# XShengTech/gpu-docker-api

Hardware: AMD Instinct MI355X
Metric: p50 replicaSet create->running + patch(GPU rescale) latency (lower is better)
Workload: dtype n/a; 1 GPU; global_batch=1, seq_len=0, parallelism=1 concurrent tenants, 1 daemon, 1 GPUs, patch=gpuCount 1->0

## Files before the change

### __graft_entry__.py

```python
from __future__ import annotations


def build() -> None:
    from gpu_docker_api_amd.ops import build as ops_build

    artifacts = ops_build.build_all()
    for name, path in artifacts.items():
        print(f"built {name}: {path}")

    import gpu_docker_api_amd
    from gpu_docker_api_amd.routers.app import build_app
    from gpu_docker_api_amd.ops import iocopy

    assert iocopy.uring_available() or True
    print("package import OK")


def smoke() -> None:
    import asyncio

    import torch

    assert torch.cuda.is_available(), "smoke() needs a GPU"

    from gpu_docker_api_amd.ops import hipcore

    ext = hipcore.load_ext()
    n = ext.device_count()
    assert n >= 1, "no HIP devices"
    info = ext.device_info(0)
    print(f"GPU0: {info['name']} ({info['gcnArchName']}), "
          f"{info['totalGlobalMem'] / 2**30:.0f} GiB")

    def err_over_bound(C, A64, B64, ref=None):
        if ref is None:
            ref = A64 @ B64
        bound = A64.shape[1] * 2.0 ** -23 * (A64.abs() @ B64.abs())
# ... 98 lines not shown
```

### gpu_docker_api_amd/ops/__init__.py

```python
"""Native ops: HIP/CDNA4 kernels and the io_uring copy engine.

Built in-tree by :mod:`.build` (the .so files live next to this file so they
travel to GPU boxes with the repo snapshot). On a GPU box these MUST load —
ops fail loudly rather than falling back to a silent eager path.
"""
```

### gpu_docker_api_amd/ops/build.py

```python
from __future__ import annotations

import os
import subprocess
import sys
import sysconfig

ROOT = os.path.dirname(os.path.dirname(os.path.dirname(os.path.abspath(__file__))))
CSRC = os.path.join(ROOT, "csrc")
OPS = os.path.join(ROOT, "gpu_docker_api_amd", "ops")
BIN = os.path.join(CSRC, "bin")
HIPCC = os.environ.get("HIPCC", "/opt/rocm/bin/hipcc")
ARCH = os.environ.get("PYTORCH_ROCM_ARCH", "gfx950")


def _newer(out: str, *srcs: str) -> bool:
    if not os.path.exists(out):
        return False
    omt = os.path.getmtime(out)
    return all(os.path.getmtime(s) <= omt for s in srcs)


def _run(cmd: list[str]) -> None:
    print("+", " ".join(cmd), flush=True)
    subprocess.run(cmd, check=True)
# ... 47 lines not shown
    src = os.path.join(CSRC, "iocopy.cpp")
    out = os.path.join(OPS, "_iocopy.so")
    if not force and _newer(out, src):
        return out
    import pybind11

    py_inc = sysconfig.get_paths()["include"]
    cmd = [
        "g++",
        "-O2",
        "-std=c++17",
        "-fPIC",
        "-shared",
        src,
        "-o",
        out,
        f"-I{pybind11.get_include()}",
        f"-I{py_inc}",
    ]
    _run(cmd)
    return out


def build_rccl_smoke(force: bool = False) -> str:
    src = os.path.join(CSRC, "rccl_smoke.hip")
    out = os.path.join(BIN, "rccl_smoke")
    if not force and _newer(out, src):
        return out
    os.makedirs(BIN, exist_ok=True)
    cmd = [
        HIPCC,
        f"--offload-arch={ARCH}",
        "-O2",
        "-std=c++17",
        src,
        "-o",
        out,
        "-I/opt/rocm/include",
        "-L/opt/rocm/lib",
        "-lrccl",
    ]
    _run(cmd)
    return out


def build_all(force: bool = False) -> dict:
    return {
        "iocopy": build_iocopy(force),
        "hipcore": build_hipcore(force),
        "rccl_smoke": build_rccl_smoke(force),
    }


if __name__ == "__main__":
    force = "--force" in sys.argv
    for name, path in build_all(force).items():
        print(f"built {name}: {path}")
```

### gpu_docker_api_amd/runtime/proc.py

```python
from __future__ import annotations

import asyncio
import json
import logging
import os
import shutil
import signal
import subprocess
import time
import uuid as uuidlib
from typing import Dict, List, Optional

from ..models.etcd import ContainerSpec
from ..utils.names import safe_subpath
from ..xerrors import ContainerExisted, ContainerNotExist, VolumeExisted
from .base import ContainerState, GpuResolver, RuntimeDriver, VolumeState
from .devices import visible_device_env

log = logging.getLogger(__name__)

CGROUP_ROOT = "/sys/fs/cgroup"
DEFAULT_CMD = ["sleep", "infinity"]


class _Proc:
    def __init__(self, state: ContainerState, spec: ContainerSpec) -> None:
        self.state = state
        self.spec = spec
        self.popen: Optional[subprocess.Popen] = None
        self.cgroup: Optional[str] = None
        self.restart_policy: str = (
            (spec.host_config.get("RestartPolicy") or {}).get("Name", "") or "no"
        )
        self.manually_stopped = False
        self.restarts = 0
        self.next_restart_at = 0.0
        self.last_start_at = 0.0
        self.attached_pid = 0
        self.attached_start = 0
        self.was_started = False
        self.start_ticks = 0


class ProcRuntime(RuntimeDriver):
    owns_rootfs = True

    def __init__(
        self,
        base_dir: str = "",
        gpu_resolver: Optional[GpuResolver] = None,
        use_cgroups: bool = True,
        loop_volumes: bool = False,
    ) -> None:
        self.base = base_dir or os.path.join(os.getcwd(), ".state", "procrt")
        for sub in ("containers", "volumes", "images", "trash"):
            os.makedirs(os.path.join(self.base, sub), exist_ok=True)
        self.gpu_resolver: GpuResolver = gpu_resolver or (lambda _u: None)
        self.use_cgroups = use_cgroups
        self.loop_volumes = loop_volumes
        self._procs: Dict[str, _Proc] = {}
        self.volumes: Dict[str, VolumeState] = {}
        self._supervisor: Optional[asyncio.Task] = None

        self._load_volumes()
        self._load_containers()
        try:
            asyncio.get_running_loop()
            if self._procs:
                self._ensure_supervisor()
        except RuntimeError:
            pass

    def _ensure_supervisor(self) -> None:
        if self._supervisor is None or self._supervisor.done():
            self._supervisor = asyncio.get_running_loop().create_task(
                self._supervise_loop()
# ... 95 lines not shown

    def _leader_pid(self, p: _Proc) -> int:
        if p.popen is not None:
            return p.popen.pid
        return p.attached_pid

    def _refresh(self, p: _Proc) -> None:
        if p.state.running and not self._alive(p):
            p.state.running = False
            p.state.status = "exited"
            p.state.pid = 0
            p.attached_pid = 0
            self._write_meta(p)

    def _write_meta(self, p: _Proc) -> None:
        try:
            meta = {
                "id": p.state.id,
                "pid": self._leader_pid(p) if p.state.running else 0,
                "starttime": p.start_ticks if p.state.running else 0,
                "running": p.state.running,
                "restarts": p.restarts,
            }
            with open(os.path.join(self._cdir(p.state.name), "meta.json"), "w") as f:
                json.dump(meta, f)
        except OSError:
            pass

    def _load_containers(self) -> None:
        trash = os.path.join(self.base, "trash")
        for entry in os.listdir(trash):
            shutil.rmtree(os.path.join(trash, entry), ignore_errors=True)
        croot = os.path.join(self.base, "containers")
        for name in sorted(os.listdir(croot)):
            if ".deleting-" in name:
                shutil.rmtree(os.path.join(croot, name), ignore_errors=True)
                continue
            specf = os.path.join(croot, name, "spec.json")
            if not os.path.isfile(specf):
                continue
            try:
                spec = ContainerSpec.deserialize(open(specf).read())
            except Exception:
                continue
            meta = {}
            try:
                meta = json.load(open(os.path.join(croot, name, "meta.json")))
            except Exception:
# ... 22 lines not shown
                    p.start_ticks = p.attached_start
                    p.was_started = True
                    p.last_start_at = time.monotonic()
                    st.pid = pid
                    st.running = True
                    state_char = self._proc_stat(pid)[0]
                    if state_char in ("T", "t"):
                        st.paused, st.status = True, "paused"
                    else:
                        st.status = "running"
                else:
                    p.restarts = 0
                    p.was_started = True
                    p.manually_stopped = False
            else:
                p.manually_stopped = True
            self._procs[name] = p

    async def create(self, spec: ContainerSpec) -> str:
        name = spec.container_name
        if name in self._procs:
            raise ContainerExisted(name)
        cid = uuidlib.uuid4().hex[:12]
        rootfs = os.path.join(self._cdir(name), "rootfs")
        os.makedirs(rootfs, exist_ok=True)
        seed = self._image_dir(spec.image) if spec.image else ""
        if seed and os.path.isdir(seed):
            await asyncio.get_running_loop().run_in_executor(
                None, lambda: shutil.copytree(seed, rootfs, dirs_exist_ok=True)
            )
        binds = list(spec.host_config.get("Binds") or [])
        for b in binds:
            src, _, dest = b.partition(":")
            dest = dest.split(":")[0]
            if not src or not dest:
                continue
            vol = self.volumes.get(src)
            src_path = vol.mountpoint if vol else src
            link = os.path.join(rootfs, dest.lstrip("/"))
            os.makedirs(os.path.dirname(link), exist_ok=True)
            if not os.path.lexists(link):
                os.symlink(src_path, link)
        st = ContainerState(
            id=cid,
            name=name,
            image=spec.image,
            status="created",
            env=list(spec.env),
            gpu_uuids=list(spec.gpu_uuids),
            cpuset_cpus=spec.cpuset_cpus,
            memory=spec.memory_bytes,
            port_bindings=dict(spec.host_config.get("PortBindings") or {}),
            upper_dir=rootfs,
            binds=binds,
        )
        p = _Proc(st, spec)
        self._procs[name] = p
        with open(os.path.join(self._cdir(name), "spec.json"), "w") as f:
            f.write(spec.serialize())
        return cid

    def _get(self, name: str) -> _Proc:
        if name not in self._procs:
            raise ContainerNotExist(name)
        return self._procs[name]

    _base_env: Optional[Dict[str, str]] = None

    def _env_for(self, p: _Proc) -> Dict[str, str]:
        if ProcRuntime._base_env is None:
            ProcRuntime._base_env = dict(os.environ)
        env = dict(ProcRuntime._base_env)
        env.update(visible_device_env(p.state.gpu_uuids, self.gpu_resolver))
        for e in p.state.env:
            k, _, v = e.partition("=")
            env[k] = v
        return env

    @staticmethod
    def _enable_controllers(path: str) -> None:
        ctrl_file = os.path.join(path, "cgroup.subtree_control")
        avail_file = os.path.join(path, "cgroup.controllers")
        try:
            with open(avail_file) as f:
                avail = set(f.read().split())
            want = [c for c in ("memory", "cpuset") if c in avail]
            for c in want:
                try:
                    with open(ctrl_file, "w") as f:
                        f.write(f"+{c}")
                except OSError:
                    pass
        except OSError:
            pass

    def _setup_cgroup(self, name: str, p: _Proc, pid: int) -> None:
        if not self.use_cgroups:
            return
        parent = os.path.join(CGROUP_ROOT, "gda")
        cg = os.path.join(parent, name)
# ... 9 lines not shown
                with open(os.path.join(cg, "cpuset.cpus"), "w") as f:
                    f.write(p.state.cpuset_cpus)
            mems = p.spec.host_config.get("CpusetMems", "")
            if mems:
                try:
                    with open(os.path.join(cg, "cpuset.mems"), "w") as f:
                        f.write(mems)
                except OSError:
                    pass
            with open(os.path.join(cg, "cgroup.procs"), "w") as f:
                f.write(str(pid))
            p.cgroup = cg
        except OSError:
            p.cgroup = None

    async def start(self, name: str) -> None:
        p = self._get(name)
        self._refresh(p)
        p.manually_stopped = False
        self._ensure_supervisor()
        if p.state.running:
            return
        cmd = list(p.spec.config.get("Cmd") or []) or DEFAULT_CMD
        logf = open(os.path.join(self._cdir(name), "console.log"), "ab")
        try:
            p.popen = subprocess.Popen(
                cmd,
                cwd=p.state.upper_dir,
                env=self._env_for(p),
                stdout=logf,
                stderr=subprocess.STDOUT,
                start_new_session=True,
            )
        finally:
            logf.close()
        p.attached_pid = 0
        p.was_started = True
        p.last_start_at = time.monotonic()
        p.start_ticks = self._proc_starttime(p.popen.pid) or 0
        p.state.pid = p.popen.pid
        p.state.running, p.state.paused, p.state.status = True, False, "running"
        self._setup_cgroup(name, p, p.popen.pid)
        self._write_meta(p)

    def _signal_group(self, p: _Proc, sig: int) -> None:
        if not self._alive(p):
            return
        try:
            os.killpg(os.getpgid(self._leader_pid(p)), sig)
        except ProcessLookupError:
            pass

    async def stop(self, name: str, timeout: int = 10, _removing: bool = False) -> None:
        p = self._get(name)
        p.manually_stopped = True
        self._refresh(p)
        if self._alive(p):
            self._signal_group(p, signal.SIGTERM)
            self._signal_group(p, signal.SIGCONT)
            spin_until = time.monotonic() + 0.002
            while time.monotonic() < spin_until and self._alive(p):
                await asyncio.sleep(0)
            deadline = time.monotonic() + timeout
            delay = 0.001
            while time.monotonic() < deadline and self._alive(p):
                await asyncio.sleep(delay)
                delay = min(delay * 2, 0.02)
            if self._alive(p):
                self._signal_group(p, signal.SIGKILL)
                kill_deadline = time.monotonic() + 5
                while time.monotonic() < kill_deadline and self._alive(p):
                    await asyncio.sleep(0.005)
        leader = self._leader_pid(p)
        if leader:
            try:
                os.killpg(leader, signal.SIGKILL)
            except (ProcessLookupError, PermissionError):
                pass
        p.state.running, p.state.paused, p.state.status = False, False, "exited"
        p.state.pid = 0
        p.attached_pid = 0
        if not _removing:
            self._write_meta(p)

    async def pause(self, name: str) -> None:
        p = self._get(name)
        if p.cgroup:
            try:
                with open(os.path.join(p.cgroup, "cgroup.freeze"), "w") as f:
                    f.write("1")
                p.state.paused, p.state.status = True, "paused"
                return
            except OSError:
                pass
        self._signal_group(p, signal.SIGSTOP)
        p.state.paused, p.state.status = True, "paused"

    async def unpause(self, name: str) -> None:
        p = self._get(name)
        if p.cgroup:
            try:
                with open(os.path.join(p.cgroup, "cgroup.freeze"), "w") as f:
                    f.write("0")
                p.state.paused, p.state.status = False, "running"
                return
            except OSError:
                pass
        self._signal_group(p, signal.SIGCONT)
        p.state.paused, p.state.status = False, "running"

    async def restart(self, name: str, timeout: int = 10) -> None:
        await self.stop(name, timeout)
        await self.start(name)

    async def remove(self, name: str, force: bool = True) -> None:
        p = self._get(name)
        self._refresh(p)
        if p.state.running:
            if not force:
                raise RuntimeError(f"{name} is running")
            await self.stop(name, timeout=2, _removing=True)
        if p.cgroup:
            try:
                os.rmdir(p.cgroup)
            except OSError:
                pass
        self._procs.pop(name, None)
        cdir = self._cdir(name)
        shutil.rmtree(cdir, ignore_errors=True)

    async def inspect(self, name: str) -> Optional[ContainerState]:
        p = self._procs.get(name)
        if p is None:
            return None
        self._refresh(p)
        return p.state

    async def list(self, all: bool = True) -> List[ContainerState]:
        for p in self._procs.values():
            self._refresh(p)
        return [p.state for p in self._procs.values() if all or p.state.running]

    async def execute_rc(self, name: str, cmd: List[str], workdir: str = ""):
        p = self._get(name)
        self._refresh(p)
        if not p.state.running:
            raise RuntimeError(f"{name} is not running")
        cwd = (
            os.path.join(p.state.upper_dir, workdir.lstrip("/"))
            if workdir
            else p.state.upper_dir
        )
# ... 172 lines not shown
```

### gpu_docker_api_amd/services/replicaset.py

```python
from __future__ import annotations

import asyncio
import logging
import os
import shutil
from typing import Dict, List, Optional, Tuple

from ..config import Config
from ..models import ContainerCommit, ContainerExecute, ContainerRun, PatchRequest
from ..models.etcd import ContainerSpec, HistoryItem, _now_str
from ..models.memory import to_bytes
from ..parallel import CpuScheduler, GpuScheduler, PortScheduler
from ..runtime.base import ContainerState, RuntimeDriver
from ..state.keys import Resource
from ..state.store import StateStore
from ..state.workqueue import WorkQueue
from ..utils.copy import CopyEngine
from ..utils.names import safe_subpath
from ..utils.timing import PhaseTimer
from ..state.keys import RELEASED_SET_KEY
from ..version import MergeMap, ReleasedSet, VersionMap
from ..xerrors import (
    ContainerExisted,
    ContainerNotExist,
    NoPatchRequired,
    NoRollbackRequired,
)
from .saga import Saga

log = logging.getLogger(__name__)


def versioned(name: str, version: int) -> str:
    return f"{name}-{version}"


class ReplicaSetService:
    def __init__(
        self,
        *,
# ... 252 lines not shown
        vname_old: str,
        timer: PhaseTimer,
        migrate_src: Optional[str] = None,
    ) -> Tuple[str, str]:
        old_state = await self.runtime.inspect(vname_old)
        cid, vname_new = await self._run_container(saga, name, spec, only_create=True, timer=timer)
        new_state = await self.runtime.inspect(vname_new)
        src = migrate_src or (old_state.upper_dir if old_state is not None else "")
        if (
            new_state is not None
            and src
            and new_state.upper_dir
            and os.path.isdir(src)
        ):
            await self.copy.copy_dir(src, new_state.upper_dir)
        timer.mark("copy")
        await self.runtime.start(vname_new)
        timer.mark("start")
        if old_state is not None and old_state.upper_dir and os.path.isdir(old_state.upper_dir):
            merge_path = safe_subpath(self.cfg.merges_dir, name, vname_old)
            try:
                if getattr(self.runtime, "owns_rootfs", False):
                    os.makedirs(os.path.dirname(merge_path), exist_ok=True)
                    shutil.rmtree(merge_path, ignore_errors=True)
                    try:
                        os.rename(old_state.upper_dir, merge_path)
                    except OSError:
                        os.makedirs(merge_path, exist_ok=True)
                        await self.copy.copy_dir(old_state.upper_dir, merge_path)
                else:
                    os.makedirs(merge_path, exist_ok=True)
                    await self.copy.copy_dir(old_state.upper_dir, merge_path)
                self.merges.set(vname_old, merge_path)
                self._prune_merge_layers(name)
            except Exception:
                log.exception("preserving %s layer failed", vname_old)
        timer.mark("preserve")
        if old_state is not None:
            self.ports.restore(self._host_ports(old_state))
            await self.runtime.remove(vname_old, force=True)
        self._released.discard(vname_old)
        timer.mark("delete_old")
        return vname_new, cid

    def _prune_merge_layers(self, name: str) -> None:
        keep = self.cfg.keep_merge_layers
        if keep <= 0:
            return
        prefix = name + "-"
        entries = []
        for vname, path in self.merges.snapshot().items():
            if vname.startswith(prefix):
                try:
                    entries.append((int(vname[len(prefix):]), vname, path))
                except ValueError:
                    continue
        entries.sort(reverse=True)
        for _v, vname, path in entries[keep:]:
            self.merges.remove(vname)
            shutil.rmtree(path, ignore_errors=True)

    @staticmethod
    def _host_ports(state: ContainerState) -> List[int]:
        out: List[int] = []
        for _cport, bindings in (state.port_bindings or {}).items():
            for b in bindings or []:
                try:
                    out.append(int(b.get("HostPort", "0")))
                except (TypeError, ValueError):
                    continue
        return [p for p in out if p]

    async def rollback_container(
        self, name: str, target_version: int, restore_data: bool = False
    ) -> Dict:
        timer = PhaseTimer("replicaset.rollback")
        cur_version = self.versions.get(name)
        if cur_version is None:
            raise ContainerNotExist(name)
        if cur_version == target_version:
            raise NoRollbackRequired(name)
        target = await self._spec_at_version(name, target_version)
        live = await self._load_spec(name)
# ... 194 lines not shown
```

### gpu_docker_api_amd/utils/files.py

```python
from __future__ import annotations

import os


def dir_size(path: str) -> int:
    total = 0
    for root, _dirs, files in os.walk(path):
        for f in files:
            fp = os.path.join(root, f)
            try:
                st = os.lstat(fp)
            except OSError:
                continue
            blocks = getattr(st, "st_blocks", None)
            total += blocks * 512 if blocks is not None else st.st_size
    return total


def is_dir(path: str) -> bool:
    return os.path.isdir(path)
```

Measured before the change: 3.846 ms.

## Move container process lifecycle to native vfork/pidfd module

Adds a pybind11 C++ module that spawns container processes with vfork/execve using a pre-encoded base environment, exposes a pidfd, and provides native tree removal and container-dir preparation. Stop now waits on the pidfd through the event loop instead of sleep-polling, and rmtree calls go through the native remover. The aim is to cut subprocess.Popen fork/exec overhead, polling latency and Python filesystem walking on the create and rescale path. It adds a native build dependency and subtle signal, fd and orphan-reaping logic. Pause also gains a short wait for the stopped state, which may add latency.

```diff
diff --git a/__graft_entry__.py b/__graft_entry__.py
--- a/__graft_entry__.py
+++ b/__graft_entry__.py
@@ -10,9 +10,10 @@
 
     import gpu_docker_api_amd
     from gpu_docker_api_amd.routers.app import build_app
-    from gpu_docker_api_amd.ops import iocopy
+    from gpu_docker_api_amd.ops import iocopy, proclife
 
     assert iocopy.uring_available() or True
+    assert proclife.available(), "native lifecycle module did not load"
     print("package import OK")
 
 
diff --git a/csrc/proclife.cpp b/csrc/proclife.cpp
--- /dev/null
+++ b/csrc/proclife.cpp
@@ -0,0 +1,151 @@
+#include <pybind11/pybind11.h>
+#include <pybind11/stl.h>
+
+#include <cstdio>
+#include <memory>
+
+#include "proclife_core.h"
+
+namespace py = pybind11;
+namespace pl = proclife;
+
+namespace {
+
+pl::BaseEnv g_base_env;
+
+std::string fsbytes(py::handle h, const char* what) {
+  PyObject* raw = nullptr;
+  if (!PyUnicode_FSConverter(h.ptr(), &raw)) throw py::error_already_set();
+  py::bytes b = py::reinterpret_steal<py::bytes>(raw);
+  std::string s = b;
+  if (s.find('\0') != std::string::npos)
+    throw py::value_error(std::string("embedded null byte in ") + what);
+  return s;
+}
+
+std::vector<pl::KV> env_items(py::handle mapping) {
+  std::vector<pl::KV> out;
+  if (mapping.is_none()) return out;
+  py::object items = py::isinstance<py::dict>(mapping)
+                         ? py::reinterpret_borrow<py::dict>(mapping).attr("items")()
+                         : py::reinterpret_borrow<py::object>(mapping);
+  for (py::handle it : items) {
+    py::tuple kv = py::reinterpret_borrow<py::tuple>(it);
+    std::string k = fsbytes(kv[0], "environment");
+    if (k.find('=') != std::string::npos)
+      throw py::value_error("illegal environment variable name");
+    out.emplace_back(std::move(k), fsbytes(kv[1], "environment"));
+  }
+  return out;
+}
+
+[[noreturn]] void raise_oserror(int err, const std::string& filename) {
+  errno = err;
+  if (filename.empty())
+    PyErr_SetFromErrno(PyExc_OSError);
+  else
+    PyErr_SetFromErrnoWithFilename(PyExc_OSError, filename.c_str());
+  throw py::error_already_set();
+}
+
+class PyChild {
+ public:
+  explicit PyChild(pl::Child&& c) : c_(std::move(c)), pid_(c_.pid) {}
+
+  int pid() const { return pid_; }
+  unsigned long long starttime() const { return c_.starttime; }
+  py::object returncode() const {
+    return c_.exited ? py::cast(c_.returncode) : py::none();
+  }
+  py::object poll() {
+    return c_.poll() ? py::cast(c_.returncode) : py::none();
+  }
+  py::object wait(py::object timeout) {
+    int ms = timeout.is_none() ? -1 : static_cast<int>(timeout.cast<double>() * 1000.0);
+    bool done;
+    {
+      py::gil_scoped_release nogil;
+      done = c_.wait(ms);
+    }
+    return done ? py::cast(c_.returncode) : py::none();
+  }
+  int fileno() const { return c_.pidfd; }
+  void close() { c_.close_fd(); }
+
+ private:
+  pl::Child c_;
+  int pid_;
+};
+
+std::unique_ptr<PyChild> spawn(py::sequence argv, py::object cwd, py::object env_overrides,
+                               py::object log_path) {
+  std::vector<std::string> args;
+  for (py::handle a : argv) args.push_back(fsbytes(a, "argv"));
+  if (args.empty()) throw py::value_error("empty argv");
+  std::string cwd_s = fsbytes(cwd, "cwd"), log_s = fsbytes(log_path, "log_path");
+  std::vector<pl::KV> over = env_items(env_overrides);
+  pl::Child child;
+  pl::SpawnError res;
+  {
+    py::gil_scoped_release nogil;
+    res = pl::spawn(args, cwd_s, g_base_env, over, log_s, &child);
+  }
+  if (res.err) raise_oserror(res.err, res.filename);
+  return std::make_unique<PyChild>(std::move(child));
+}
+
+}
+
+PYBIND11_MODULE(_proclife, m) {
+  m.doc() = "container process lifecycle on raw syscalls (csrc/proclife_core.h)";
+
+  py::class_<PyChild>(m, "Child")
+      .def_property_readonly("pid", &PyChild::pid)
+      .def_property_readonly("starttime", &PyChild::starttime)
+      .def_property_readonly("returncode", &PyChild::returncode)
+      .def("poll", &PyChild::poll)
+      .def("wait", &PyChild::wait, py::arg("timeout") = py::none())
+      .def("fileno", &PyChild::fileno)
+      .def("close", &PyChild::close);
+
+  m.def(
+      "set_base_env",
+      [](py::object mapping) {
+        g_base_env.set(env_items(mapping));
+        return g_base_env.size();
+      },
+      py::arg("env"), "snapshot and encode the base environment once");
+  m.def("base_env_size", [] { return g_base_env.size(); });
+  m.def("spawn", &spawn, py::arg("argv"), py::arg("cwd"), py::arg("env_overrides"),
+        py::arg("log_path"));
+  m.def("proc_starttime", [](int pid) { return pl::read_starttime(pid); }, py::arg("pid"));
+  m.def(
+      "remove_tree",
+      [](py::object path) {
+        std::string p = fsbytes(path, "path");
+        long failed;
+        {
+          py::gil_scoped_release nogil;
+          failed = pl::remove_tree(p.c_str());
+        }
+        return failed;
+      },
+      py::arg("path"));
+  m.def(
+      "prepare_container_dir",
+      [](py::object cdir, py::object spec_json) {
+        std::string d = fsbytes(cdir, "cdir"), failed;
+        std::string data = spec_json.cast<std::string>();
+        if (int e = pl::prepare_container_dir(d, data.data(), data.size(), &failed))
+          raise_oserror(e, failed);
+      },
+      py::arg("cdir"), py::arg("spec_json"));
+  m.def(
+      "write_file",
+      [](py::object path, py::object data) {
+        std::string p = fsbytes(path, "path");
+        std::string d = data.cast<std::string>();
+        if (int e = pl::write_file(p.c_str(), d.data(), d.size())) raise_oserror(e, p);
+      },
+      py::arg("path"), py::arg("data"));
+}
diff --git a/csrc/proclife_core.h b/csrc/proclife_core.h
--- /dev/null
+++ b/csrc/proclife_core.h
@@ -0,0 +1,515 @@
+#pragma once
+
+#ifndef _GNU_SOURCE
+#define _GNU_SOURCE
+#endif
+
+#include <cerrno>
+#include <cstdio>
+#include <csignal>
+#include <cstdlib>
+#include <cstring>
+#include <mutex>
+#include <string>
+#include <unordered_map>
+#include <utility>
+#include <vector>
+
+#include <dirent.h>
+#include <fcntl.h>
+#include <poll.h>
+#include <sys/stat.h>
+#include <sys/syscall.h>
+#include <sys/types.h>
+#include <sys/wait.h>
+#include <unistd.h>
+
+namespace proclife {
+
+using KV = std::pair<std::string, std::string>;
+
+
+class BaseEnv {
+ public:
+  void set(const std::vector<KV>& kv) {
+    entries_.clear();
+    index_.clear();
+    entries_.reserve(kv.size());
+    for (const auto& e : kv) {
+      auto it = index_.find(e.first);
+      if (it == index_.end()) {
+        index_.emplace(e.first, entries_.size());
+        entries_.push_back(e.first + "=" + e.second);
+      } else {
+        entries_[it->second] = e.first + "=" + e.second;
+      }
+    }
+  }
+  size_t size() const { return entries_.size(); }
+  const std::vector<std::string>& entries() const { return entries_; }
+  long find(const std::string& key) const {
+    auto it = index_.find(key);
+    return it == index_.end() ? -1 : static_cast<long>(it->second);
+  }
+
+ private:
+  std::vector<std::string> entries_;
+  std::unordered_map<std::string, size_t> index_;
+};
+
+class MergedEnv {
+ public:
+  MergedEnv(const BaseEnv& base, const std::vector<KV>& overrides) {
+    const auto& be = base.entries();
+    slots_.reserve(be.size() + overrides.size() + 1);
+    for (const auto& s : be) slots_.push_back(s.c_str());
+    owned_.reserve(overrides.size());
+    std::vector<std::pair<const std::string*, size_t>> added;
+    for (const auto& o : overrides) {
+      owned_.push_back(o.first + "=" + o.second);
+      const char* entry = owned_.back().c_str();
+      long at = base.find(o.first);
+      if (at < 0) {
+        for (const auto& a : added)
+          if (*a.first == o.first) at = static_cast<long>(a.second);
+      }
+      if (at >= 0) {
+        slots_[static_cast<size_t>(at)] = entry;
+      } else {
+        added.emplace_back(&o.first, slots_.size());
+        slots_.push_back(entry);
+      }
+    }
+    slots_.push_back(nullptr);
+  }
+  char* const* envp() const { return const_cast<char* const*>(slots_.data()); }
+  const char* get(const char* key) const {
+    size_t n = std::strlen(key);
+    for (const char* e : slots_)
+      if (e && std::strncmp(e, key, n) == 0 && e[n] == '=') return e + n + 1;
+    return nullptr;
+  }
+
+ private:
+  std::vector<std::string> owned_;
+  std::vector<const char*> slots_;
+};
+
+
+inline unsigned long long read_starttime(pid_t pid, char* state_out = nullptr) {
+  char path[48];
+  std::snprintf(path, sizeof path, "/proc/%d/stat", static_cast<int>(pid));
+  int fd = ::open(path, O_RDONLY | O_CLOEXEC);
+  if (fd < 0) return 0;
+  char buf[2048];
+  size_t len = 0;
+  for (;;) {
+    ssize_t n = ::read(fd, buf + len, sizeof buf - 1 - len);
+    if (n < 0 && errno == EINTR) continue;
+    if (n <= 0) break;
+    len += static_cast<size_t>(n);
+    if (len == sizeof buf - 1) break;
+  }
+  ::close(fd);
+  buf[len] = '\0';
+  const char* after = nullptr;
+  for (size_t i = 0; i + 1 < len; ++i)
+    if (buf[i] == ')' && buf[i + 1] == ' ') after = buf + i + 2;
+  if (!after) return 0;
+  char state = *after;
+  if (state_out) *state_out = state;
+  if (state == 'Z' || state == 'X' || state == '\0') return 0;
+  const char* p = after;
+  for (int field = 0; field < 19; ++field) {
+    while (*p && *p != ' ' && *p != '\n') ++p;
+    while (*p == ' ') ++p;
+    if (!*p) return 0;
+  }
+  char* end = nullptr;
+  errno = 0;
+  unsigned long long v = std::strtoull(p, &end, 10);
+  if (end == p || errno) return 0;
+  return v;
+}
+
+
+#ifndef P_PIDFD
+#define P_PIDFD 3
+#endif
+
+namespace detail {
+inline std::mutex& orphan_mu() {
+  static std::mutex m;
+  return m;
+}
+inline std::vector<pid_t>& orphans() {
+  static std::vector<pid_t> v;
+  return v;
+}
+inline void reap_orphans() {
+  std::lock_guard<std::mutex> g(orphan_mu());
+  auto& v = orphans();
+  for (size_t i = 0; i < v.size();) {
+    int st;
+    pid_t r = ::waitpid(v[i], &st, WNOHANG);
+    if (r == v[i] || (r < 0 && errno == ECHILD)) {
+      v[i] = v.back();
+      v.pop_back();
+    } else {
+      ++i;
+    }
+  }
+}
+}
+
+struct Child {
+  pid_t pid = -1;
+  int pidfd = -1;
+  unsigned long long starttime = 0;
+  bool exited = false;
+  int returncode = 0;
+
+  Child() = default;
+  Child(const Child&) = delete;
+  Child& operator=(const Child&) = delete;
+  Child(Child&& o) noexcept { *this = std::move(o); }
+  Child& operator=(Child&& o) noexcept {
+    if (this != &o) {
+      release();
+      pid = o.pid, pidfd = o.pidfd, starttime = o.starttime;
+      exited = o.exited, returncode = o.returncode;
+      o.pid = -1, o.pidfd = -1, o.exited = true;
+    }
+    return *this;
+  }
+  ~Child() { release(); }
+
+  bool poll() {
+    if (exited || pid <= 0) return exited;
+    siginfo_t info;
+    for (;;) {
+      std::memset(&info, 0, sizeof info);
+      int r = pidfd >= 0
+                  ? ::waitid(static_cast<idtype_t>(P_PIDFD), static_cast<id_t>(pidfd), &info,
+                             WEXITED | WNOHANG)
+                  : ::waitid(P_PID, static_cast<id_t>(pid), &info, WEXITED | WNOHANG);
+      if (r == 0) break;
+      if (errno == EINTR) continue;
+      exited = true;
+      returncode = 0;
+      return true;
+    }
+    if (info.si_pid == 0) return false;
+    exited = true;
+    returncode = info.si_code == CLD_EXITED ? info.si_status : -info.si_status;
+    return true;
+  }
+
+  bool wait(int timeout_ms) {
+    if (poll()) return true;
+    if (pidfd >= 0) {
+      struct pollfd pfd = {pidfd, POLLIN, 0};
+      for (;;) {
+        int r = ::poll(&pfd, 1, timeout_ms);
+        if (r < 0 && errno == EINTR) continue;
+        break;
+      }
+      return poll();
+    }
+    for (int waited = 0; timeout_ms < 0 || waited < timeout_ms; ++waited) {
+      if (poll()) return true;
+      ::usleep(1000);
+    }
+    return poll();
+  }
+
+  void close_fd() {
+    if (pidfd >= 0) {
+      ::close(pidfd);
+      pidfd = -1;
+    }
+  }
+
+  void release() {
+    if (pid > 0 && !exited && !poll()) {
+      std::lock_guard<std::mutex> g(detail::orphan_mu());
+      detail::orphans().push_back(pid);
+    }
+    close_fd();
+    pid = -1;
+  }
+};
+
+
+struct SpawnError {
+  int err = 0;
+  std::string filename;
+};
+
+namespace detail {
+
+#ifndef SYS_close_range
+#define SYS_close_range 436
+#endif
+
+struct ChildPlan {
+  int logfd;
+  const char* cwd;
+  char* const* argv;
+  char* const* envp;
+  const char* const* candidates;
+  const sigset_t* sigmask;
+  int max_fd;
+  volatile int* err;
+  volatile int* stage;
+};
+
+[[noreturn]] __attribute__((noinline)) inline void child_exec(const ChildPlan& p) {
+  struct sigaction dfl;
+  std::memset(&dfl, 0, sizeof dfl);
+  dfl.sa_handler = SIG_DFL;
+  for (int sig = 1; sig < NSIG; ++sig) {
+    struct sigaction cur;
+    if (::sigaction(sig, nullptr, &cur) != 0 || cur.sa_handler == SIG_DFL) continue;
+    if (cur.sa_handler == SIG_IGN && sig != SIGPIPE && sig != SIGXFSZ) continue;
+    ::sigaction(sig, &dfl, nullptr);
+  }
+  int stage = 3;
+  do {
+    if (::setsid() < 0) break;
+    if (::dup2(p.logfd, 1) < 0 || ::dup2(p.logfd, 2) < 0) break;
+    stage = 1;
+    if (::chdir(p.cwd) != 0) break;
+    stage = 3;
+    if (::sigprocmask(SIG_SETMASK, p.sigmask, nullptr) != 0) break;
+    if (::syscall(SYS_close_range, 3U, ~0U, 0U) != 0)
+      for (int fd = 3; fd < p.max_fd; ++fd) ::close(fd);
+    stage = 2;
+    int saved = 0;
+    for (const char* const* c = p.candidates; *c; ++c) {
+      ::execve(*c, p.argv, p.envp);
+      if (errno != ENOENT && errno != ENOTDIR && saved == 0) saved = errno;
+    }
+    if (saved) errno = saved;
+  } while (false);
+  *p.err = errno ? errno : EINVAL;
+  *p.stage = stage;
+  ::_exit(127);
+}
+
+__attribute__((noinline)) inline pid_t vfork_child(const ChildPlan& plan, int* vfork_errno) {
+  pid_t pid = ::vfork();
+  if (pid == 0) child_exec(plan);
+  *vfork_errno = errno;
+  return pid;
+}
+
+}
+
+inline SpawnError spawn(const std::vector<std::string>& argv, const std::string& cwd,
+                        const BaseEnv& base, const std::vector<KV>& overrides,
+                        const std::string& log_path, Child* out) {
+  SpawnError res;
+  if (argv.empty()) {
+    res.err = EINVAL;
+    return res;
+  }
+  detail::reap_orphans();
+  MergedEnv env(base, overrides);
+
+  std::vector<char*> cargv;
+  cargv.reserve(argv.size() + 1);
+  for (const auto& a : argv) cargv.push_back(const_cast<char*>(a.c_str()));
+  cargv.push_back(nullptr);
+
+  std::vector<std::string> cands;
+  int skipped_err = ENOENT;
+  const std::string& name = argv[0];
+  if (name.find('/') != std::string::npos) {
+    cands.push_back(name);
+  } else {
+    const char* path = env.get("PATH");
+    std::string dirs = path ? path : "/bin:/usr/bin";
+    for (size_t pos = 0;;) {
+      size_t colon = dirs.find(':', pos);
+      std::string dir = dirs.substr(pos, colon == std::string::npos ? colon : colon - pos);
+      std::string cand = dir.empty() ? name : dir + "/" + name;
+      std::string probe = cand[0] == '/' ? cand : cwd + "/" + cand;
+      struct stat st;
+      if (::stat(probe.c_str(), &st) != 0 && (errno == ENOENT || errno == ENOTDIR))
+        skipped_err = errno;
+      else
+        cands.push_back(std::move(cand));
+      if (colon == std::string::npos) break;
+      pos = colon + 1;
+    }
+  }
+  std::vector<const char*> cptrs;
+  cptrs.reserve(cands.size() + 1);
+  for (const auto& c : cands) cptrs.push_back(c.c_str());
+  cptrs.push_back(nullptr);
+
+  int logfd = ::open(log_path.c_str(), O_WRONLY | O_CREAT | O_APPEND | O_CLOEXEC, 0666);
+  if (logfd < 0) {
+    res.err = errno, res.filename = log_path;
+    return res;
+  }
+  if (logfd < 3) {
+    int moved = ::fcntl(logfd, F_DUPFD_CLOEXEC, 3);
+    int e = errno;
+    ::close(logfd);
+    if (moved < 0) {
+      res.err = e, res.filename = log_path;
+      return res;
+    }
+    logfd = moved;
+  }
+
+  volatile int child_err = 0, child_stage = 0;
+  pid_t pid = -1;
+  int err = 0;
+  if (cands.empty()) {
+    struct stat st;
+    if (::stat(cwd.c_str(), &st) != 0) {
+      err = errno, child_stage = 1;
+    } else {
+      err = skipped_err, child_stage = 2;
+    }
+  } else {
+    long open_max = ::sysconf(_SC_OPEN_MAX);
+    sigset_t all, old;
+    sigfillset(&all);
+    pthread_sigmask(SIG_SETMASK, &all, &old);
+    detail::ChildPlan plan = {logfd,        cwd.c_str(), cargv.data(),
+                              env.envp(),   cptrs.data(), &old,
+                              open_max > 0 && open_max < 65536 ? static_cast<int>(open_max) : 65536,
+                              &child_err,   &child_stage};
+    int vfork_err = 0;
+    pid = detail::vfork_child(plan, &vfork_err);
+    pthread_sigmask(SIG_SETMASK, &old, nullptr);
+    if (pid < 0) {
+      err = vfork_err, child_stage = 3;
+    } else if (child_err != 0) {
+      err = child_err;
+      int st;
+      while (::waitpid(pid, &st, 0) < 0 && errno == EINTR) {
+      }
+    }
+  }
+  ::close(logfd);
+
+  if (err != 0) {
+    res.err = err;
+    res.filename = child_stage == 1 ? cwd : child_stage == 2 ? argv[0] : std::string();
+    return res;
+  }
+  Child c;
+  c.pid = pid;
+  c.pidfd = static_cast<int>(::syscall(SYS_pidfd_open, pid, 0));
+  c.starttime = read_starttime(pid);
+  *out = std::move(c);
+  return res;
+}
+
+
+namespace detail {
+
+constexpr int kDirFlags = O_RDONLY | O_DIRECTORY | O_NOFOLLOW | O_CLOEXEC;
+
+inline long empty_dir(int dfd) {
+  DIR* d = ::fdopendir(dfd);
+  if (!d) {
+    ::close(dfd);
+    return 1;
+  }
+  std::vector<std::pair<std::string, unsigned char>> names;
+  for (;;) {
+    errno = 0;
+    struct dirent* e = ::readdir(d);
+    if (!e) break;
+    const char* n = e->d_name;
+    if (n[0] == '.' && (n[1] == '\0' || (n[1] == '.' && n[2] == '\0'))) continue;
+    names.emplace_back(n, e->d_type);
+  }
+  long failed = errno ? 1 : 0;
+  for (auto& ent : names) {
+    const char* n = ent.first.c_str();
+    bool is_dir = ent.second == DT_DIR;
+    if (ent.second == DT_UNKNOWN) {
+      struct stat st;
+      is_dir = ::fstatat(dfd, n, &st, AT_SYMLINK_NOFOLLOW) == 0 && S_ISDIR(st.st_mode);
+    }
+    if (is_dir) {
+      int sub = ::openat(dfd, n, kDirFlags);
+      if (sub < 0) {
+        ++failed;
+        continue;
+      }
+      failed += empty_dir(sub);
+      if (::unlinkat(dfd, n, AT_REMOVEDIR) != 0) ++failed;
+    } else if (::unlinkat(dfd, n, 0) != 0) {
+      ++failed;
+    }
+  }
+  ::closedir(d);
+  return failed;
+}
+
+}
+
+inline long remove_tree(const char* path) {
+  int dfd = ::open(path, detail::kDirFlags);
+  if (dfd < 0) return errno == ENOENT ? 0 : 1;
+  long failed = detail::empty_dir(dfd);
+  if (::rmdir(path) != 0) ++failed;
+  return failed;
+}
+
+
+inline int write_file(const char* path, const char* data, size_t len) {
+  int fd = ::open(path, O_WRONLY | O_CREAT | O_TRUNC | O_CLOEXEC, 0666);
+  if (fd < 0) return errno;
+  while (len > 0) {
+    ssize_t n = ::write(fd, data, len);
+    if (n < 0) {
+      if (errno == EINTR) continue;
+      int e = errno;
+      ::close(fd);
+      return e;
+    }
+    data += n, len -= static_cast<size_t>(n);
+  }
+  return ::close(fd) != 0 ? errno : 0;
+}
+
+inline int make_dirs(const std::string& path) {
+  if (::mkdir(path.c_str(), 0777) == 0) return 0;
+  if (errno == EEXIST) {
+    struct stat st;
+    return (::stat(path.c_str(), &st) == 0 && S_ISDIR(st.st_mode)) ? 0 : EEXIST;
+  }
+  if (errno != ENOENT) return errno;
+  size_t end = path.find_last_not_of('/');
+  size_t slash = end == std::string::npos ? end : path.rfind('/', end);
+  if (slash == std::string::npos || slash == 0) return ENOENT;
+  if (int e = make_dirs(path.substr(0, slash))) return e;
+  if (::mkdir(path.c_str(), 0777) == 0 || errno == EEXIST) return 0;
+  return errno;
+}
+
+inline int prepare_container_dir(const std::string& cdir, const char* spec, size_t len,
+                                 std::string* failed) {
+  std::string rootfs = cdir + "/rootfs";
+  if (int e = make_dirs(rootfs)) {
+    *failed = rootfs;
+    return e;
+  }
+  std::string specf = cdir + "/spec.json";
+  if (int e = write_file(specf.c_str(), spec, len)) {
+    *failed = specf;
+    return e;
+  }
+  return 0;
+}
+
+}
diff --git a/csrc/proclife_selftest.cpp b/csrc/proclife_selftest.cpp
--- /dev/null
+++ b/csrc/proclife_selftest.cpp
@@ -0,0 +1,217 @@
+#include <cstdio>
+#include <cstdlib>
+#include <fstream>
+#include <sstream>
+
+#include "proclife_core.h"
+
+namespace pl = proclife;
+
+static int g_failed = 0;
+#define CHECK(cond)                                                        \
+  do {                                                                     \
+    if (!(cond)) {                                                         \
+      std::fprintf(stderr, "FAIL %s:%d: %s\n", __FILE__, __LINE__, #cond); \
+      ++g_failed;                                                          \
+    }                                                                      \
+  } while (0)
+
+static int count_fds() {
+  DIR* d = ::opendir("/proc/self/fd");
+  if (!d) return -1;
+  int n = 0;
+  while (struct dirent* e = ::readdir(d))
+    if (e->d_name[0] != '.') ++n;
+  ::closedir(d);
+  return n - 1;
+}
+
+static bool have_children() {
+  siginfo_t info;
+  std::memset(&info, 0, sizeof info);
+  return ::waitid(P_ALL, 0, &info, WEXITED | WNOHANG | WNOWAIT) == 0;
+}
+
+static std::string slurp(const std::string& path) {
+  std::ifstream f(path);
+  std::stringstream ss;
+  ss << f.rdbuf();
+  return ss.str();
+}
+
+static void build_tree(const std::string& root) {
+  CHECK(pl::make_dirs(root + "/a/b/c") == 0);
+  CHECK(pl::write_file((root + "/a/f1").c_str(), "x", 1) == 0);
+  CHECK(pl::write_file((root + "/a/b/f2").c_str(), "yy", 2) == 0);
+  CHECK(::link((root + "/a/f1").c_str(), (root + "/a/b/c/hard").c_str()) == 0);
+  CHECK(::symlink("/nonexistent/target", (root + "/a/dangling").c_str()) == 0);
+  CHECK(pl::write_file((root + "/locked").c_str(), "z", 1) == 0);
+  CHECK(::chmod((root + "/locked").c_str(), 0) == 0);
+}
+
+int main() {
+  char tmpl[] = "/tmp/proclife-selftest-XXXXXX";
+  const char* made = ::mkdtemp(tmpl);
+  if (!made) {
+    std::perror("mkdtemp");
+    return 2;
+  }
+  const std::string top = made;
+
+  pl::BaseEnv base;
+  base.set({{"PATH", "/usr/local/bin:/usr/bin:/bin"}, {"KEEP", "1"}, {"OVER", "base"}});
+
+  { pl::Child warm; }
+  const int fds_before = count_fds();
+  CHECK(!have_children());
+
+  {
+    pl::MergedEnv env(base, {{"OVER", "a=b"}, {"NEW", ""}, {"NEW", "last"}, {"OVER", "final"}});
+    CHECK(std::string(env.get("OVER")) == "final");
+    CHECK(std::string(env.get("NEW")) == "last");
+    CHECK(std::string(env.get("KEEP")) == "1");
+    CHECK(env.get("ABSENT") == nullptr);
+    int n = 0;
+    for (char* const* e = env.envp(); *e; ++e) ++n;
+    CHECK(n == 4);
+  }
+
+  for (int round = 0; round < 200; ++round) {
+    const std::string cdir = top + "/c" + std::to_string(round);
+    std::string failed;
+    CHECK(pl::prepare_container_dir(cdir, "{}", 2, &failed) == 0);
+    pl::Child c;
+    pl::SpawnError e = pl::spawn({"sleep", "30"}, cdir + "/rootfs", base,
+                                 {{"ROUND", std::to_string(round)}}, cdir + "/console.log", &c);
+    CHECK(e.err == 0);
+    if (e.err) break;
+    CHECK(c.pid > 0 && c.pidfd >= 0 && c.starttime > 0);
+    CHECK(::getsid(c.pid) == c.pid && ::getpgid(c.pid) == c.pid);
+    CHECK(!c.poll());
+    CHECK(pl::read_starttime(c.pid) == c.starttime);
+    if (round % 3 == 0) {
+      CHECK(::kill(-c.pid, SIGKILL) == 0);
+    } else {
+      CHECK(::kill(-c.pid, round % 2 ? SIGTERM : SIGKILL) == 0);
+      CHECK(c.wait(5000));
+      CHECK(c.returncode == (round % 2 ? -SIGTERM : -SIGKILL));
+      CHECK(c.poll() && c.poll());
+      c.close_fd();
+      c.close_fd();
+    }
+    CHECK(pl::remove_tree(cdir.c_str()) == 0);
+    struct stat st;
+    CHECK(::lstat(cdir.c_str(), &st) != 0 && errno == ENOENT);
+  }
+
+  {
+    const std::string cdir = top + "/out";
+    std::string failed;
+    CHECK(pl::prepare_container_dir(cdir, "{}", 2, &failed) == 0);
+    for (int i = 0; i < 2; ++i) {
+      pl::Child c;
+      pl::SpawnError e = pl::spawn({"sh", "-c", "echo out; echo err >&2; exit 7"}, cdir + "/rootfs",
+                                   base, {}, cdir + "/console.log", &c);
+      CHECK(e.err == 0);
+      CHECK(c.wait(5000) && c.returncode == 7);
+    }
+    CHECK(slurp(cdir + "/console.log") == "out\nerr\nout\nerr\n");
+    CHECK(pl::remove_tree(cdir.c_str()) == 0);
+  }
+
+  {
+    const std::string cdir = top + "/bad";
+    std::string failed;
+    CHECK(pl::prepare_container_dir(cdir, "{}", 2, &failed) == 0);
+    CHECK(pl::write_file((cdir + "/rootfs/noexec").c_str(), "#!/bin/sh\n", 10) == 0);
+    CHECK(::chmod((cdir + "/rootfs/noexec").c_str(), 0644) == 0);
+    for (int round = 0; round < 200; ++round) {
+      pl::Child c;
+      pl::SpawnError e;
+      switch (round % 5) {
+        case 0:
+          e = pl::spawn({"definitely-not-a-command"}, cdir + "/rootfs", base, {},
+                        cdir + "/console.log", &c);
+          CHECK(e.err == ENOENT);
+          break;
+        case 1:
+          e = pl::spawn({"./noexec"}, cdir + "/rootfs", base, {}, cdir + "/console.log", &c);
+          CHECK(e.err == EACCES);
+          break;
+        case 2:
+          e = pl::spawn({"/no/such/binary"}, cdir + "/rootfs", base, {}, cdir + "/console.log", &c);
+          CHECK(e.err == ENOENT);
+          break;
+        case 3:
+          e = pl::spawn({"sleep", "1"}, cdir + "/missing-cwd", base, {}, cdir + "/console.log", &c);
+          CHECK(e.err == ENOENT && e.filename == cdir + "/missing-cwd");
+          break;
+        default:
+          e = pl::spawn({"sleep", "1"}, cdir + "/rootfs", base, {}, cdir + "/no-dir/console.log",
+                        &c);
+          CHECK(e.err == ENOENT);
+          break;
+      }
+      CHECK(c.pid == -1 && c.pidfd == -1);
+    }
+    CHECK(pl::remove_tree(cdir.c_str()) == 0);
+  }
+
+  for (int round = 0; round < 50; ++round) {
+    const std::string root = top + "/tree";
+    build_tree(root);
+    CHECK(pl::remove_tree(root.c_str()) == 0);
+    struct stat st;
+    CHECK(::lstat(root.c_str(), &st) != 0);
+  }
+  {
+    const std::string outside = top + "/outside", root = top + "/tree2";
+    CHECK(pl::make_dirs(outside) == 0 && pl::make_dirs(root) == 0);
+    CHECK(pl::write_file((outside + "/keep").c_str(), "k", 1) == 0);
+    CHECK(::symlink(outside.c_str(), (root + "/link").c_str()) == 0);
+    CHECK(pl::remove_tree(root.c_str()) == 0);
+    CHECK(slurp(outside + "/keep") == "k");
+    CHECK(::symlink(outside.c_str(), (top + "/rootlink").c_str()) == 0);
+    CHECK(pl::remove_tree((top + "/rootlink").c_str()) == 1);
+    CHECK(slurp(outside + "/keep") == "k");
+    CHECK(::unlink((top + "/rootlink").c_str()) == 0);
+    CHECK(pl::remove_tree((top + "/never-existed").c_str()) == 0);
+    CHECK(pl::remove_tree(outside.c_str()) == 0);
+  }
+  {
+    const std::string root = top + "/deep", seg(100, 'd');
+    CHECK(pl::make_dirs(root) == 0);
+    int fd = ::open(root.c_str(), O_RDONLY | O_DIRECTORY | O_CLOEXEC);
+    CHECK(fd >= 0);
+    for (int level = 0; level < 60 && fd >= 0; ++level) {
+      CHECK(::mkdirat(fd, seg.c_str(), 0777) == 0);
+      int file = ::openat(fd, "f", O_WRONLY | O_CREAT | O_CLOEXEC, 0666);
+      CHECK(file >= 0);
+      if (file >= 0) ::close(file);
+      int next = ::openat(fd, seg.c_str(), O_RDONLY | O_DIRECTORY | O_CLOEXEC);
+      ::close(fd);
+      fd = next;
+    }
+    if (fd >= 0) ::close(fd);
+    CHECK(pl::remove_tree(root.c_str()) == 0);
+    struct stat st;
+    CHECK(::lstat(root.c_str(), &st) != 0);
+  }
+
+  pl::detail::reap_orphans();
+  for (int i = 0; i < 200 && have_children(); ++i) {
+    ::usleep(5000);
+    pl::detail::reap_orphans();
+  }
+  CHECK(!have_children());
+  CHECK(pl::detail::orphans().empty());
+  CHECK(count_fds() == fds_before);
+  CHECK(pl::remove_tree(top.c_str()) == 0);
+
+  if (g_failed) {
+    std::fprintf(stderr, "proclife selftest: %d check(s) FAILED\n", g_failed);
+    return 1;
+  }
+  std::printf("proclife selftest OK\n");
+  return 0;
+}
diff --git a/gpu_docker_api_amd/ops/__init__.py b/gpu_docker_api_amd/ops/__init__.py
--- a/gpu_docker_api_amd/ops/__init__.py
+++ b/gpu_docker_api_amd/ops/__init__.py
@@ -1,4 +1,5 @@
-"""Native ops: HIP/CDNA4 kernels and the io_uring copy engine.
+"""Native ops: HIP/CDNA4 kernels, the io_uring copy engine and the proc
+runtime's lifecycle module (spawn / reap / teardown).
 
 Built in-tree by :mod:`.build` (the .so files live next to this file so they
 travel to GPU boxes with the repo snapshot). On a GPU box these MUST load —
diff --git a/gpu_docker_api_amd/ops/build.py b/gpu_docker_api_amd/ops/build.py
--- a/gpu_docker_api_amd/ops/build.py
+++ b/gpu_docker_api_amd/ops/build.py
@@ -93,6 +93,31 @@
     return out
 
 
+def build_proclife(force: bool = False) -> str:
+    src = os.path.join(CSRC, "proclife.cpp")
+    core = os.path.join(CSRC, "proclife_core.h")
+    out = os.path.join(OPS, "_proclife.so")
+    if not force and _newer(out, src, core):
+        return out
+    import pybind11
+
+    py_inc = sysconfig.get_paths()["include"]
+    cmd = [
+        "g++",
+        "-O2",
+        "-std=c++17",
+        "-fPIC",
+        "-shared",
+        src,
+        "-o",
+        out,
+        f"-I{pybind11.get_include()}",
+        f"-I{py_inc}",
+    ]
+    _run(cmd)
+    return out
+
+
 def build_rccl_smoke(force: bool = False) -> str:
     src = os.path.join(CSRC, "rccl_smoke.hip")
     out = os.path.join(BIN, "rccl_smoke")
@@ -118,6 +143,7 @@
 def build_all(force: bool = False) -> dict:
     return {
         "iocopy": build_iocopy(force),
+        "proclife": build_proclife(force),
         "hipcore": build_hipcore(force),
         "rccl_smoke": build_rccl_smoke(force),
     }
diff --git a/gpu_docker_api_amd/ops/proclife.py b/gpu_docker_api_amd/ops/proclife.py
--- /dev/null
+++ b/gpu_docker_api_amd/ops/proclife.py
@@ -0,0 +1,83 @@
+from __future__ import annotations
+
+import importlib.util
+import os
+from typing import Dict, Optional, Sequence
+
+ENABLED = os.environ.get("GDA_NATIVE_LIFECYCLE", "1").strip().lower() not in (
+    "0", "false", "no", "off",
+)
+
+_ext = None
+_ext_err: Optional[str] = None
+_base_env: Optional[Dict[str, str]] = None
+
+
+def _load():
+    global _ext, _ext_err
+    if _ext is not None:
+        return _ext
+    if _ext_err is not None:
+        raise ImportError(_ext_err)
+    so = os.path.join(os.path.dirname(os.path.abspath(__file__)), "_proclife.so")
+    if not os.path.exists(so):
+        _ext_err = f"{so} not built (run ops.build)"
+        raise ImportError(_ext_err)
+    try:
+        spec = importlib.util.spec_from_file_location("_proclife", so)
+        mod = importlib.util.module_from_spec(spec)
+        spec.loader.exec_module(mod)
+    except Exception as e:
+        _ext_err = f"{so} failed to load: {e}"
+        raise ImportError(_ext_err) from e
+    _ext = mod
+    return mod
+
+
+def available() -> bool:
+    try:
+        _load()
+        return True
+    except ImportError:
+        return False
+
+
+def load_error() -> Optional[str]:
+    return None if available() else _ext_err
+
+
+def enabled() -> bool:
+    return ENABLED and available()
+
+
+def set_base_env(env: Dict[str, str]) -> int:
+    global _base_env
+    n = _load().set_base_env(env)
+    _base_env = env
+    return n
+
+
+def base_env_is(env: Dict[str, str]) -> bool:
+    return _base_env is env
+
+
+def spawn(argv: Sequence[str], cwd: str, env_overrides: Dict[str, str], log_path: str):
+    if _base_env is None:
+        set_base_env(dict(os.environ))
+    return _load().spawn(list(argv), cwd, env_overrides, log_path)
+
+
+def remove_tree(path: str) -> int:
+    return _load().remove_tree(path)
+
+
+def prepare_container_dir(cdir: str, spec_json: str) -> None:
+    _load().prepare_container_dir(cdir, spec_json)
+
+
+def write_file(path: str, data) -> None:
+    _load().write_file(path, data)
+
+
+def proc_starttime(pid: int) -> int:
+    return _load().proc_starttime(pid)
diff --git a/gpu_docker_api_amd/runtime/proc.py b/gpu_docker_api_amd/runtime/proc.py
--- a/gpu_docker_api_amd/runtime/proc.py
+++ b/gpu_docker_api_amd/runtime/proc.py
@@ -12,6 +12,7 @@
 from typing import Dict, List, Optional
 
 from ..models.etcd import ContainerSpec
+from ..ops import proclife
 from ..utils.names import safe_subpath
 from ..xerrors import ContainerExisted, ContainerNotExist, VolumeExisted
 from .base import ContainerState, GpuResolver, RuntimeDriver, VolumeState
@@ -22,12 +23,17 @@
 CGROUP_ROOT = "/sys/fs/cgroup"
 DEFAULT_CMD = ["sleep", "infinity"]
 
+NATIVE_LIFECYCLE = proclife.enabled()
+if proclife.ENABLED and not NATIVE_LIFECYCLE:
+    log.warning("native lifecycle module not loaded (%s): using the Python path",
+                proclife.load_error())
+
 
 class _Proc:
     def __init__(self, state: ContainerState, spec: ContainerSpec) -> None:
         self.state = state
         self.spec = spec
-        self.popen: Optional[subprocess.Popen] = None
+        self.popen = None
         self.cgroup: Optional[str] = None
         self.restart_policy: str = (
             (spec.host_config.get("RestartPolicy") or {}).get("Name", "") or "no"
@@ -40,6 +46,7 @@
         self.attached_start = 0
         self.was_started = False
         self.start_ticks = 0
+        self.exit_waiters: List[asyncio.Future] = []
 
 
 class ProcRuntime(RuntimeDriver):
@@ -51,7 +58,11 @@
         gpu_resolver: Optional[GpuResolver] = None,
         use_cgroups: bool = True,
         loop_volumes: bool = False,
+        native: Optional[bool] = None,
     ) -> None:
+        if native is None:
+            native = NATIVE_LIFECYCLE
+        self._nat = proclife if native and proclife.available() else None
         self.base = base_dir or os.path.join(os.getcwd(), ".state", "procrt")
         for sub in ("containers", "volumes", "images", "trash"):
             os.makedirs(os.path.join(self.base, sub), exist_ok=True)
@@ -193,8 +204,12 @@
                 "running": p.state.running,
                 "restarts": p.restarts,
             }
-            with open(os.path.join(self._cdir(p.state.name), "meta.json"), "w") as f:
-                json.dump(meta, f)
+            path = os.path.join(self._cdir(p.state.name), "meta.json")
+            if self._nat is not None:
+                self._nat.write_file(path, json.dumps(meta))
+            else:
+                with open(path, "w") as f:
+                    json.dump(meta, f)
         except OSError:
             pass
 
@@ -263,14 +278,18 @@
         if name in self._procs:
             raise ContainerExisted(name)
         cid = uuidlib.uuid4().hex[:12]
-        rootfs = os.path.join(self._cdir(name), "rootfs")
-        os.makedirs(rootfs, exist_ok=True)
+        cdir = self._cdir(name)
+        rootfs = os.path.join(cdir, "rootfs")
         seed = self._image_dir(spec.image) if spec.image else ""
-        if seed and os.path.isdir(seed):
+        seeded = bool(seed) and os.path.isdir(seed)
+        binds = list(spec.host_config.get("Binds") or [])
+        one_call = self._nat is not None and not seeded and not binds
+        if not one_call:
+            os.makedirs(rootfs, exist_ok=True)
+        if seeded:
             await asyncio.get_running_loop().run_in_executor(
                 None, lambda: shutil.copytree(seed, rootfs, dirs_exist_ok=True)
             )
-        binds = list(spec.host_config.get("Binds") or [])
         for b in binds:
             src, _, dest = b.partition(":")
             dest = dest.split(":")[0]
@@ -296,9 +315,14 @@
             binds=binds,
         )
         p = _Proc(st, spec)
+        if one_call:
+            self._nat.prepare_container_dir(cdir, spec.serialize())
         self._procs[name] = p
-        with open(os.path.join(self._cdir(name), "spec.json"), "w") as f:
-            f.write(spec.serialize())
+        if self._nat is None:
+            with open(os.path.join(cdir, "spec.json"), "w") as f:
+                f.write(spec.serialize())
+        elif not one_call:
+            self._nat.write_file(os.path.join(cdir, "spec.json"), spec.serialize())
         return cid
 
     def _get(self, name: str) -> _Proc:
@@ -308,15 +332,34 @@
 
     _base_env: Optional[Dict[str, str]] = None
 
-    def _env_for(self, p: _Proc) -> Dict[str, str]:
+    @staticmethod
+    def _base_snapshot() -> Dict[str, str]:
         if ProcRuntime._base_env is None:
             ProcRuntime._base_env = dict(os.environ)
-        env = dict(ProcRuntime._base_env)
-        env.update(visible_device_env(p.state.gpu_uuids, self.gpu_resolver))
+        return ProcRuntime._base_env
+
+    def _env_overrides(self, p: _Proc) -> Dict[str, str]:
+        env = dict(visible_device_env(p.state.gpu_uuids, self.gpu_resolver))
         for e in p.state.env:
             k, _, v = e.partition("=")
             env[k] = v
         return env
+
+    def _env_for(self, p: _Proc) -> Dict[str, str]:
+        env = dict(self._base_snapshot())
+        env.update(self._env_overrides(p))
+        return env
+
+    def _spawn_native(self, name: str, p: _Proc, cmd: List[str]):
+        base = self._base_snapshot()
+        if not self._nat.base_env_is(base):
+            self._nat.set_base_env(base)
+        return self._nat.spawn(
+            cmd,
+            p.state.upper_dir,
+            self._env_overrides(p),
+            os.path.join(self._cdir(name), "console.log"),
+        )
 
     @staticmethod
     def _enable_controllers(path: str) -> None:
@@ -372,22 +415,27 @@
         if p.state.running:
             return
         cmd = list(p.spec.config.get("Cmd") or []) or DEFAULT_CMD
-        logf = open(os.path.join(self._cdir(name), "console.log"), "ab")
-        try:
-            p.popen = subprocess.Popen(
-                cmd,
-                cwd=p.state.upper_dir,
-                env=self._env_for(p),
-                stdout=logf,
-                stderr=subprocess.STDOUT,
-                start_new_session=True,
-            )
-        finally:
-            logf.close()
+        if self._nat is not None:
+            p.popen = self._spawn_native(name, p, cmd)
+            start_ticks = p.popen.starttime
+        else:
+            logf = open(os.path.join(self._cdir(name), "console.log"), "ab")
+            try:
+                p.popen = subprocess.Popen(
+                    cmd,
+                    cwd=p.state.upper_dir,
+                    env=self._env_for(p),
+                    stdout=logf,
+                    stderr=subprocess.STDOUT,
+                    start_new_session=True,
+                )
+            finally:
+                logf.close()
+            start_ticks = self._proc_starttime(p.popen.pid) or 0
         p.attached_pid = 0
         p.was_started = True
         p.last_start_at = time.monotonic()
-        p.start_ticks = self._proc_starttime(p.popen.pid) or 0
+        p.start_ticks = start_ticks
         p.state.pid = p.popen.pid
         p.state.running, p.state.paused, p.state.status = True, False, "running"
         self._setup_cgroup(name, p, p.popen.pid)
@@ -400,6 +448,48 @@
             os.killpg(os.getpgid(self._leader_pid(p)), sig)
         except ProcessLookupError:
             pass
+
+    @staticmethod
+    def _has_pidfd(p: _Proc) -> bool:
+        return p.popen is not None and not isinstance(p.popen, subprocess.Popen)
+
+    async def _await_exit(self, p: _Proc, fd: int, timeout: float) -> bool:
+        loop = asyncio.get_running_loop()
+        fut = loop.create_future()
+
+        def wake(futs) -> None:
+            for f in futs:
+                if not f.done():
+                    f.set_result(None)
+
+        waiters = p.exit_waiters
+        if not waiters:
+            loop.add_reader(fd, wake, waiters)
+        waiters.append(fut)
+        timer = loop.call_later(timeout, wake, (fut,))
+        try:
+            await fut
+        finally:
+            timer.cancel()
+            waiters.remove(fut)
+            if not waiters:
+                loop.remove_reader(fd)
+        return not self._alive(p)
+
+    async def _poll_exit(self, p: _Proc, timeout: float) -> None:
+        spin_until = time.monotonic() + 0.002
+        while time.monotonic() < spin_until and self._alive(p):
+            await asyncio.sleep(0)
+        deadline = time.monotonic() + timeout
+        delay = 0.001
+        while time.monotonic() < deadline and self._alive(p):
+            await asyncio.sleep(delay)
+            delay = min(delay * 2, 0.02)
+        if self._alive(p):
+            self._signal_group(p, signal.SIGKILL)
+            kill_deadline = time.monotonic() + 5
+            while time.monotonic() < kill_deadline and self._alive(p):
+                await asyncio.sleep(0.005)
 
     async def stop(self, name: str, timeout: int = 10, _removing: bool = False) -> None:
         p = self._get(name)
@@ -408,19 +498,13 @@
         if self._alive(p):
             self._signal_group(p, signal.SIGTERM)
             self._signal_group(p, signal.SIGCONT)
-            spin_until = time.monotonic() + 0.002
-            while time.monotonic() < spin_until and self._alive(p):
-                await asyncio.sleep(0)
-            deadline = time.monotonic() + timeout
-            delay = 0.001
-            while time.monotonic() < deadline and self._alive(p):
-                await asyncio.sleep(delay)
-                delay = min(delay * 2, 0.02)
-            if self._alive(p):
-                self._signal_group(p, signal.SIGKILL)
-                kill_deadline = time.monotonic() + 5
-                while time.monotonic() < kill_deadline and self._alive(p):
-                    await asyncio.sleep(0.005)
+            child_fd = p.popen.fileno() if self._has_pidfd(p) else -1
+            if child_fd >= 0:
+                if not await self._await_exit(p, child_fd, timeout):
+                    self._signal_group(p, signal.SIGKILL)
+                    await self._await_exit(p, child_fd, 5)
+            else:
+                await self._poll_exit(p, timeout)
         leader = self._leader_pid(p)
         if leader:
             try:
@@ -444,6 +528,11 @@
             except OSError:
                 pass
         self._signal_group(p, signal.SIGSTOP)
+        leader = self._leader_pid(p)
+        for _ in range(50):
+            if not leader or self._proc_stat(leader)[0] in ("T", "t", None):
+                break
+            await asyncio.sleep(0.002)
         p.state.paused, p.state.status = True, "paused"
 
     async def unpause(self, name: str) -> None:
@@ -477,7 +566,10 @@
                 pass
         self._procs.pop(name, None)
         cdir = self._cdir(name)
-        shutil.rmtree(cdir, ignore_errors=True)
+        if self._nat is not None:
+            self._nat.remove_tree(cdir)
+        else:
+            shutil.rmtree(cdir, ignore_errors=True)
 
     async def inspect(self, name: str) -> Optional[ContainerState]:
         p = self._procs.get(name)
diff --git a/gpu_docker_api_amd/services/replicaset.py b/gpu_docker_api_amd/services/replicaset.py
--- a/gpu_docker_api_amd/services/replicaset.py
+++ b/gpu_docker_api_amd/services/replicaset.py
@@ -16,6 +16,7 @@
 from ..state.store import StateStore
 from ..state.workqueue import WorkQueue
 from ..utils.copy import CopyEngine
+from ..utils.files import remove_tree
 from ..utils.names import safe_subpath
 from ..utils.timing import PhaseTimer
 from ..state.keys import RELEASED_SET_KEY
@@ -314,7 +315,7 @@
             try:
                 if getattr(self.runtime, "owns_rootfs", False):
                     os.makedirs(os.path.dirname(merge_path), exist_ok=True)
-                    shutil.rmtree(merge_path, ignore_errors=True)
+                    remove_tree(merge_path)
                     try:
                         os.rename(old_state.upper_dir, merge_path)
                     except OSError:
@@ -350,7 +351,7 @@
         entries.sort(reverse=True)
         for _v, vname, path in entries[keep:]:
             self.merges.remove(vname)
-            shutil.rmtree(path, ignore_errors=True)
+            remove_tree(path)
 
     @staticmethod
     def _host_ports(state: ContainerState) -> List[int]:
diff --git a/gpu_docker_api_amd/utils/files.py b/gpu_docker_api_amd/utils/files.py
--- a/gpu_docker_api_amd/utils/files.py
+++ b/gpu_docker_api_amd/utils/files.py
@@ -1,6 +1,9 @@
 from __future__ import annotations
 
 import os
+import shutil
+
+from ..ops import proclife
 
 
 def dir_size(path: str) -> int:
@@ -19,3 +22,10 @@
 
 def is_dir(path: str) -> bool:
     return os.path.isdir(path)
+
+
+def remove_tree(path: str) -> None:
+    if proclife.enabled():
+        proclife.remove_tree(path)
+    else:
+        shutil.rmtree(path, ignore_errors=True)
```

After: 3.530 ms, median of 6. 1.09x faster.
